# derinworks/penr-oz-neural-network-v3-torch-ddp

Hardware: AMD Instinct MI355X
Metric: tokens/sec (whole node) GPT-2 124M DDP train at 1/2/4/8 MI355X (higher is better)
Workload: dtype bf16; 1 GPU; model=gpt2-124m, global_batch=64, seq_len=1024, micro_batch_per_gpu=64, parallelism=dp1

## Files before the change

### csrc/bindings.cpp

```cpp
#include <torch/extension.h>
#include <hip/hip_runtime.h>
#include <tuple>
#include <vector>

void layernorm_fwd(torch::Tensor x, torch::Tensor w, torch::Tensor b, double eps, torch::Tensor y, torch::Tensor mean,
                   torch::Tensor rstd);
void add_layernorm_fwd(torch::Tensor resid_in, torch::Tensor delta, torch::Tensor resid_out, torch::Tensor w,
                       torch::Tensor b, double eps, torch::Tensor y, torch::Tensor mean, torch::Tensor rstd,
                       c10::optional<torch::Tensor> delta_bias, double dropout_p, int64_t dropout_seed);
void layernorm_bwd(torch::Tensor dy, torch::Tensor x, torch::Tensor mean, torch::Tensor rstd, torch::Tensor w,
                   torch::Tensor dresid, bool accumulate, c10::optional<torch::Tensor> dresid_bf, torch::Tensor dw,
                   torch::Tensor db, c10::optional<torch::Tensor> dbias_prev, double dropout_p, int64_t dropout_seed);
std::vector<torch::Tensor> rmsnorm_fwd(torch::Tensor x, torch::Tensor w, double eps);
std::vector<torch::Tensor> rmsnorm_bwd(torch::Tensor dy, torch::Tensor x, torch::Tensor w, torch::Tensor rstd);
std::vector<torch::Tensor> rms_residual(torch::Tensor x, torch::Tensor a, c10::optional<torch::Tensor> w1,
                                        c10::optional<torch::Tensor> w2, int64_t mode, double eps1, double eps2);
void gelu_fwd(torch::Tensor x, int64_t approx, torch::Tensor y);
void gelu_bwd(torch::Tensor dy, torch::Tensor x, int64_t approx, c10::optional<torch::Tensor> dbias, torch::Tensor out);
void colsum(torch::Tensor x, torch::Tensor out);
torch::Tensor gated_act_fwd(torch::Tensor g, torch::Tensor u, int64_t kind);
torch::Tensor gated_act_packed(torch::Tensor gu, int64_t kind, c10::optional<torch::Tensor> out);
std::vector<torch::Tensor> gated_act_bwd(torch::Tensor dy, torch::Tensor g, torch::Tensor u, int64_t kind);
void gated_act_bwd_packed(torch::Tensor dy, torch::Tensor gu, torch::Tensor dgu, int64_t kind);
void gemma_combine_fwd(int64_t mode, torch::Tensor x, c10::optional<torch::Tensor> a, c10::optional<torch::Tensor> w1,
// ... 88 lines not shown
std::tuple<torch::Tensor, torch::Tensor, torch::Tensor> token_logprobs(torch::Tensor logits, torch::Tensor tokens,
                                                                       int64_t n);
void token_logprobs_step(torch::Tensor logits, torch::Tensor idx, torch::Tensor step, torch::Tensor n_t,
                         torch::Tensor lp_buf, torch::Tensor top_id_buf, torch::Tensor top_lp_buf,
                         torch::Tensor workspace);
void stop_begin(torch::Tensor tail, torch::Tensor n_gen, torch::Tensor done, torch::Tensor finish_at);
void stop_observe(torch::Tensor seqs, torch::Tensor seq_len, torch::Tensor n_seqs, torch::Tensor tail,
                  torch::Tensor n_gen, torch::Tensor done, torch::Tensor finish_at, torch::Tensor tok);
void stop_step(torch::Tensor seqs, torch::Tensor seq_len, torch::Tensor n_seqs, torch::Tensor tail,
               torch::Tensor n_gen, torch::Tensor done, torch::Tensor finish_at, torch::Tensor idx,
               torch::Tensor out_buf, torch::Tensor step);
void logit_bias_apply(torch::Tensor logits, torch::Tensor ids, torch::Tensor bias, torch::Tensor until,
                      torch::Tensor n_entries, c10::optional<torch::Tensor> allow, bool allow_on, torch::Tensor base_t,
                      c10::optional<torch::Tensor> step_t);
std::tuple<int64_t, int64_t, int64_t> logit_bias_plan(int64_t B, int64_t V, bool allow_on);
torch::Tensor update_moments(std::vector<torch::Tensor> ws, std::vector<torch::Tensor> ps);
bool gemm_nt_supported(int64_t M, int64_t N, int64_t K);
void gemm_nt(torch::Tensor a, torch::Tensor b, c10::optional<torch::Tensor> bias, torch::Tensor out,
             c10::optional<torch::Tensor> act, int64_t approx, int64_t group_m, int64_t grid, int64_t ablate);
void wgrad_gemm(torch::Tensor dy, torch::Tensor x, torch::Tensor grad, int64_t tile, int64_t variant, bool accumulate);
void flash_attn_fwd(torch::Tensor qkv, torch::Tensor out, torch::Tensor lse, int64_t H, int64_t Hkv, int64_t D,
                    double scale, double p_drop, int64_t seed);
int64_t flash_fwd_variant(int64_t v);
void flash_bwd_stamps(c10::optional<torch::Tensor> buf);
void flash_attn_bwd(torch::Tensor dout, torch::Tensor qkv, torch::Tensor out, torch::Tensor lse, torch::Tensor dqkv,
                    int64_t H, int64_t Hkv, int64_t D, double scale, double p_drop, int64_t seed,
                    c10::optional<torch::Tensor> dbias);
void flash_attn_gen_fwd(torch::Tensor qkv, torch::Tensor out, torch::Tensor lse, int64_t H, int64_t Hkv, int64_t D,
                        double scale, double p_drop, int64_t seed);
void flash_attn_gen_bwd(torch::Tensor dout, torch::Tensor qkv, torch::Tensor out, torch::Tensor lse,
                        torch::Tensor dqkv, int64_t H, int64_t Hkv, int64_t D, double scale, double p_drop,
                        int64_t seed);
std::vector<int64_t> attn_work_plan(int64_t nblk, int64_t nvh, int64_t slots, int64_t BM, int64_t BN, int64_t T,
                                    int64_t D, double tile_us);

static int64_t cu_masked_stream(int64_t device, std::vector<int64_t> mask) {
  std::vector<uint32_t> m(mask.begin(), mask.end());
  int prev = 0;
  TORCH_CHECK(hipGetDevice(&prev) == hipSuccess, "hipGetDevice failed");
  TORCH_CHECK(hipSetDevice((int)device) == hipSuccess, "hipSetDevice failed");
  hipStream_t st = nullptr;
  const hipError_t e = hipExtStreamCreateWithCUMask(&st, (uint32_t)m.size(), m.data());
  (void)hipSetDevice(prev);
  TORCH_CHECK(e == hipSuccess, "hipExtStreamCreateWithCUMask: ", hipGetErrorString(e));
  return reinterpret_cast<int64_t>(st);
}
// ... 174 lines not shown
        pybind11::arg("nrot") = 0, pybind11::arg("cos") = pybind11::none(), pybind11::arg("sin") = pybind11::none(),
        pybind11::arg("pairs_per_wave") = 0,
        "paired-row int8-weight decode GEMV for 1..4 rows: gated MLP (mode 1) or RoPE QKV (mode 2) epilogue");
  m.def("decode_gemv_q8_limits", &decode_gemv_q8_limits,
        "(rows, K, LN-mode K, paired-row K, K multiple) limits of decode_gemv_q8 / decode_gemv_q8_pair (host only)");
  m.def("decode_gemv_q8_plan", &decode_gemv_q8_plan, pybind11::arg("M"), pybind11::arg("N"), pybind11::arg("K"),
        pybind11::arg("ln") = false, pybind11::arg("rows_per_wave") = 0,
        "decode_gemv_q8's launch plan: (form 0 half-wave / 1 wave-per-row / 2 LN, rows, row pairs per wave, "
        "chunks per lane, grid) (host only)");
  m.def("decode_gemv_q8_pair_plan", &decode_gemv_q8_pair_plan, pybind11::arg("N"), pybind11::arg("K"),
        pybind11::arg("pairs_per_wave") = 0,
        "decode_gemv_q8_pair's launch plan: (pairs per wave, chunks per lane, grid) (host only)");
  m.def("update_moments", &update_moments, "per-epoch weight-update diagnostics: [n, 2] (std(w - prev), std(w))");
  m.def("gemm_nt_supported", &gemm_nt_supported, "shapes the native NT GEMM takes (M % 256, N % 128, K % 32, K >= 160)");
  m.def("gemm_nt", &gemm_nt, pybind11::arg("a"), pybind11::arg("b"), pybind11::arg("bias"), pybind11::arg("out"),
        pybind11::arg("act") = pybind11::none(), pybind11::arg("approx") = 0, pybind11::arg("group_m") = 0,
        pybind11::arg("grid") = 0, pybind11::arg("ablate") = 0,
        "out = a·bᵀ (+ bias) (bf16, both operands reduction-contiguous); with act: act = GELU(out)");
  m.def("wgrad_gemm", &wgrad_gemm, pybind11::arg("dy"), pybind11::arg("x"), pybind11::arg("grad"),
        pybind11::arg("tile") = 256, pybind11::arg("variant") = 8, pybind11::arg("accumulate") = true,
        "grad (+)= dyᵀ·x (fp32 gradient, bf16 operands); accumulate=False overwrites grad");
  m.def("flash_attn_fwd", &flash_attn_fwd);
  m.def("flash_fwd_variant", &flash_fwd_variant, pybind11::arg("variant") = 0,
        "select the forward kernel (1 single-stage, 2 tile-pipelined); returns the previous one");
  m.def("flash_attn_bwd", &flash_attn_bwd, pybind11::arg("dout"), pybind11::arg("qkv"), pybind11::arg("out"),
        pybind11::arg("lse"), pybind11::arg("dqkv"), pybind11::arg("H"), pybind11::arg("Hkv"), pybind11::arg("D"),
        pybind11::arg("scale"), pybind11::arg("p_drop"), pybind11::arg("seed"), pybind11::arg("dbias") = pybind11::none(),
        "causal flash-attention backward (head_dim 64) into dqkv; dbias += column sums of dqkv when given");
  m.def("cu_masked_stream", &cu_masked_stream, "stream restricted to a CU mask (raw hipStream_t)");
  m.def("cu_count", &cu_count, "compute units of a device");
  m.def("flash_bwd_stamps", &flash_bwd_stamps, pybind11::arg("buf") = pybind11::none(),
        "diagnostic: s_memtime phase sums of the dK/dV kernel into an int64 [6] GPU tensor (None: off)");
  m.def("flash_attn_gen_fwd", &flash_attn_gen_fwd, "causal flash attention forward, head_dim 128 / 256");
  m.def("flash_attn_gen_bwd", &flash_attn_gen_bwd, "causal flash attention backward, head_dim 128 / 256");
}
```

### csrc/kernels/flash_attn.hip

```cpp
#include "attn_common.h"
#include <cstdlib>
#include "deferred.h"
#include <type_traits>
#include <torch/extension.h>
#include <ATen/hip/HIPContext.h>

namespace penroz {

constexpr int kD = 64;

template <bool DROPOUT>
__global__ void __launch_bounds__(256, 2) fa_fwd_kernel(const bf16* __restrict__ qkv, bf16* __restrict__ out,
                                                     float* __restrict__ lse, int T, int H, int Hkv, float scale,
                                                     float p_drop, uint64_t seed) {
  constexpr int BM = 128, BN = 64;
  __shared__ __attribute__((aligned(16))) char smem[2][2][BN * 128];
  const int nqb = (T + BM - 1) / BM;
  int qi, bh;
  xcd_head_block(qi, bh);
  const int qb = nqb - 1 - qi;
  const int b = bh / H, h = bh % H, hk = h / (H / Hkv);
  const int lane = threadIdx.x & 63, w = wave_id(), hh = lane >> 5;
  const size_t RS = (size_t)(H + 2 * Hkv) * kD;
  const bf16* qbase = qkv + (size_t)b * T * RS + (size_t)h * kD;
  const bf16* kbase = qkv + (size_t)b * T * RS + (size_t)(H + hk) * kD;
// ... 108 lines not shown
        for (int ss = 0; ss < 2; ++ss) {
          const uint4 pf = acc_frag(s[kh], ss);
#pragma unroll
          for (int dh = 0; dh < 2; ++dh) o[dh] = mfma32(tr_frag(Vt, 32 * kh + 16 * ss, 32 * dh, lane), pf, o[dh]);
        }
    }
    if (j + 1 < ntiles) lstore((j + 1) & 1);
    __syncthreads();
  }
  l = halves_sum(l);
  const float inv = l > 0.f ? 1.f / l : 0.f;
  if (qrow < T) {
    bf16* orow = out + ((size_t)b * T + qrow) * H * kD + (size_t)h * kD;
#pragma unroll
    for (int dh = 0; dh < 2; ++dh)
#pragma unroll
      for (int g = 0; g < 4; ++g)
        store4(orow + 32 * dh + 8 * g + 4 * hh, o[dh][4 * g] * inv, o[dh][4 * g + 1] * inv, o[dh][4 * g + 2] * inv,
               o[dh][4 * g + 3] * inv);
    if (hh == 0) lse[((size_t)b * H + h) * T + qrow] = (m + log2f(l)) * kLn2;
  }
}

template <bool DROPOUT>
__global__ void __launch_bounds__(128, 2) fa_fwd3_kernel(const bf16* __restrict__ qkv, bf16* __restrict__ out,
                                                      float* __restrict__ lse, int T, int H, int Hkv, float scale,
                                                      float p_drop, uint64_t seed) {
  constexpr int BM = 128, BN = 64;
  __shared__ __attribute__((aligned(16))) char smem[2][2][BN * 128];
  const int nqb = (T + BM - 1) / BM;
  int qi, bh;
  xcd_head_block(qi, bh);
  const int qb = nqb - 1 - qi;
  const int b = bh / H, h = bh % H, hk = h / (H / Hkv);
  const int lane = threadIdx.x & 63, w = wave_id(), hh = lane >> 5;
  const size_t RS = (size_t)(H + 2 * Hkv) * kD;
  const bf16* qbase = qkv + (size_t)b * T * RS + (size_t)h * kD;
  const bf16* kbase = qkv + (size_t)b * T * RS + (size_t)(H + hk) * kD;
  const bf16* vbase = qkv + (size_t)b * T * RS + (size_t)(H + Hkv + hk) * kD;
  const int q0 = qb * BM + 64 * w;
  const float c = scale * kLog2e;
  const float inv_keep = DROPOUT ? 1.f / (1.f - p_drop) : 1.f;
  int qrow[2];
  qrow[0] = q0 + (lane & 31);
  qrow[1] = q0 + 32 + (lane & 31);

  uint4 qf[2][4];
#pragma unroll
  for (int a = 0; a < 2; ++a)
#pragma unroll
    for (int s = 0; s < 4; ++s)
      qf[a][s] = qrow[a] < T ? *reinterpret_cast<const uint4*>(qbase + (size_t)qrow[a] * RS + 16 * s + 8 * hh) : zero4();
#pragma unroll
  for (int a = 0; a < 2; ++a)
#pragma unroll
    for (int s = 0; s < 4; ++s) launder(qf[a][s]);

  const unsigned RSB = (unsigned)RS * 2;
  const unsigned k_voff = (unsigned)lane * RSB;
  unsigned v_voff[2];
#pragma unroll
  for (int par = 0; par < 2; ++par) {
    const int row = 8 * par + (lane >> 3);
    const int ch = (lane & 7) ^ ((((row >> 1) & 1) << 2) | ((row >> 2) & 3));
    v_voff[par] = (unsigned)(lane >> 3) * RSB + 16u * ch;
  }
  unsigned vto[2][2];
#pragma unroll
  for (int dh = 0; dh < 2; ++dh)
#pragma unroll
    for (int jj = 0; jj < 2; ++jj) {
      const int col = 32 * dh + 16 * ((lane >> 4) & 1) + 4 * (lane & 3);
      vto[dh][jj] = (unsigned)(tile_off(4 * hh + ((lane & 15) >> 2) + 8 * jj, col >> 3) + ((col & 4) << 1));
    }
  auto vfrag = [&](const char* t, int dh) -> uint4 {
    const s16x4 x = __builtin_amdgcn_ds_read_tr16_b64_v4i16((lds_s16x4*)(t + vto[dh][0]));
    const s16x4 y = __builtin_amdgcn_ds_read_tr16_b64_v4i16((lds_s16x4*)(t + vto[dh][1]));
    const uint2 ux = __builtin_bit_cast(uint2, x), uy = __builtin_bit_cast(uint2, y);
    return uint4{ux.x, ux.y, uy.x, uy.y};
  };
  auto dma = [&](int kt0, int buf) {
    const unsigned dst = __builtin_amdgcn_readfirstlane(lds_addr_of(smem[buf][w]));
    if (kt0 + BN <= T) {
      if (w == 0) {
        const char* sb = reinterpret_cast<const char*>(kbase + (size_t)kt0 * RS);
#pragma unroll
        for (int p = 0; p < 8; ++p) glds16_s(sb + 16 * p, k_voff, dst + p * 1024);
      } else {
#pragma unroll
        for (int p = 0; p < 8; ++p)
          glds16_s(reinterpret_cast<const char*>(vbase + (size_t)(kt0 + 8 * p) * RS), v_voff[p & 1],
                      dst + p * 1024);
      }
    } else if (w == 0) {
      const bf16* g = kbase + (size_t)min(kt0 + lane, T - 1) * RS;
#pragma unroll
      for (int p = 0; p < 8; ++p) glds16(g + 8 * p, dst + p * 1024);
    } else {
      const int prow = lane >> 3, pch = lane & 7;
#pragma unroll
      for (int p = 0; p < 8; ++p) {
        const int row = 8 * p + prow;
        const int ch = pch ^ ((((row >> 1) & 1) << 2) | ((row >> 2) & 3));
        glds16(vbase + (size_t)min(kt0 + row, T - 1) * RS + 8 * ch, dst + p * 1024);
      }
    }
  };

  const int kend = min(T, qb * BM + BM);
  const int ntiles = (kend + BN - 1) / BN;
  const int jlast = min(ntiles - 1, q0 / BN);
  f32x16 o[2][2];
#pragma unroll
  for (int a = 0; a < 2; ++a)
#pragma unroll
    for (int dh = 0; dh < 2; ++dh)
#pragma unroll
      for (int i = 0; i < 16; ++i) o[a][dh][i] = 0.f;
  float m[2] = {-1e30f, -1e30f}, l[2] = {0.f, 0.f};

  auto softmax = [&](auto mask_tag, int a, int kt0, f32x16 (&sa)[2]) {
    constexpr bool MASK = decltype(mask_tag)::value;
    float tmax = -INFINITY;
#pragma unroll
    for (int kh = 0; kh < 2; ++kh)
#pragma unroll
      for (int i = 0; i < 16; ++i) {
// ... 123 lines not shown
  const int row = gid >> 3, part = gid & 7;
  const bool ok = row < B * T * H;
  float s = 0.f;
  if (ok) {
    float a[8], o[8];
    Vec8<bf16>::load(dout + (size_t)row * kD + 8 * part, a);
    Vec8<bf16>::load(out + (size_t)row * kD + 8 * part, o);
#pragma unroll
    for (int k = 0; k < 8; ++k) s += a[k] * o[k];
  }
  s += __shfl_xor(s, 1, 64);
  s += __shfl_xor(s, 2, 64);
  s += __shfl_xor(s, 4, 64);
  if (ok && part == 0) {
    const int h = row % H, t = (row / H) % T, b = row / (H * T);
    delta[((size_t)b * H + h) * T + t] = s;
  }
}

template <int NST>
struct RingWait {
  template <int PER>
  static __device__ __forceinline__ void wait() {
    static_assert(NST >= 3 && NST <= 4 && (PER == 4 || PER == 5), "ring depth / pieces");
    if constexpr (NST == 3) {
      if constexpr (PER == 4) asm volatile("s_waitcnt vmcnt(4)" ::: "memory");
      else asm volatile("s_waitcnt vmcnt(5)" ::: "memory");
    } else {
      if constexpr (PER == 4) asm volatile("s_waitcnt vmcnt(8)" ::: "memory");
      else asm volatile("s_waitcnt vmcnt(10)" ::: "memory");
    }
  }
};

template <typename F, int... S>
__device__ __forceinline__ void ring_unroll(F&& f, int base, std::integer_sequence<int, S...>) {
  (f(base + S, std::integral_constant<int, S>{}), ...);
}
template <typename F, int... S>
__device__ __forceinline__ void ring_tail(F&& f, int base, int total, std::integer_sequence<int, S...>) {
  ((base + S < total ? f(base + S, std::integral_constant<int, S>{}) : void()), ...);
}

__device__ __forceinline__ uint32_t bf16_hilo(float x) {
  const float hi = __bfloat162float(__float2bfloat16(x));
  return pack_bf16x2(hi, x - hi);
}

template <bool DROPOUT, int NST, int GC, bool STAMP = false>
__global__ void __launch_bounds__(256, 2) fa_bwd_dkdv3_kernel(const bf16* __restrict__ qkv,
                                                              const bf16* __restrict__ dout,
                                                              const float* __restrict__ lse,
                                                              const float* __restrict__ delta,
                                                              bf16* __restrict__ dqkv, float* __restrict__ cpart, int T, int H, int Hkv,
                                                              float scale, float p_drop, uint64_t seed,
                                                              unsigned long long* __restrict__ stamps = nullptr,
                                                              int diag = 0) {
  unsigned long long st_acc[5] = {0, 0, 0, 0, 0}, st_n = 0, st_t = 0;
  auto stamp = [&](int seg) {
    if constexpr (STAMP) {
      __builtin_amdgcn_sched_barrier(0);
      const unsigned long long now = __builtin_amdgcn_s_memtime();
      if (seg >= 0) st_acc[seg] += now - st_t;
      st_t = now;
      __builtin_amdgcn_sched_barrier(0);
    }
  };
  constexpr int BK = 128, QS = 64;
  constexpr int TILE = QS * 128;
  constexpr int STAGE = 2 * TILE + 512;
  __shared__ __attribute__((aligned(16))) char smem[NST * STAGE];
  int kb, bh;
  xcd_head_block(kb, bh);
  const int b = bh / Hkv, hk = bh % Hkv;
  const int G = GC ? GC : H / Hkv;
  const int lane = threadIdx.x & 63, w = wave_id(), hh = lane >> 5;
  const size_t RS = (size_t)(H + 2 * Hkv) * kD;
  const size_t ORS = (size_t)H * kD;
  const int kw0 = kb * BK + 32 * w;
  const int key = kw0 + (lane & 31);
  const uint32_t dkey = DROPOUT ? dropout_seedmix(seed) ^ ((uint32_t)(key >> 1) * kDropKeyMul) : 0u;
  const uint32_t dthr = dropout_thr(p_drop);
  const float c = scale * kLog2e;
  const float inv_keep = DROPOUT ? 1.f / (1.f - p_drop) : 1.f;

  const bf16* kbase = qkv + (size_t)b * T * RS + (size_t)(H + hk) * kD;
  const bf16* vbase = qkv + (size_t)b * T * RS + (size_t)(H + Hkv + hk) * kD;
  uint4 kf[4], vf[4];
#pragma unroll
  for (int s = 0; s < 4; ++s) {
    kf[s] = key < T ? *reinterpret_cast<const uint4*>(kbase + (size_t)key * RS + 16 * s + 8 * hh) : zero4();
// ... 17 lines not shown
  unsigned ro[4], to[2][2];
#pragma unroll
  for (int s = 0; s < 4; ++s) ro[s] = (unsigned)tile_off(lane & 31, 2 * s + hh);
#pragma unroll
  for (int dh = 0; dh < 2; ++dh)
#pragma unroll
    for (int j = 0; j < 2; ++j) {
      const int col = 32 * dh + 16 * ((lane >> 4) & 1) + 4 * (lane & 3);
      to[dh][j] = (unsigned)(tile_off(4 * hh + ((lane & 15) >> 2) + 8 * j, col >> 3) + ((col & 4) << 1));
    }
  auto rowf = [&](const char* t, int s) -> uint4 { return *reinterpret_cast<const uint4*>(t + ro[s]); };
  auto trf = [&](const char* t, int dh) -> uint4 {
    const s16x4 x = __builtin_amdgcn_ds_read_tr16_b64_v4i16((lds_s16x4*)(t + to[dh][0]));
    const s16x4 y = __builtin_amdgcn_ds_read_tr16_b64_v4i16((lds_s16x4*)(t + to[dh][1]));
    const uint2 ux = __builtin_bit_cast(uint2, x), uy = __builtin_bit_cast(uint2, y);
    return uint4{ux.x, ux.y, uy.x, uy.y};
  };

  const int s_first = (kb * BK) / QS;
  const int nslices = (T + QS - 1) / QS;
  const int per_head = nslices - s_first;
  const int total = G * per_head;

  const int is_do = w >> 1, half_sel = w & 1;
  const unsigned rsb = (unsigned)(is_do ? ORS : RS) * 2;
  unsigned voff[2];
#pragma unroll
  for (int par = 0; par < 2; ++par) {
    const int row = 8 * par + (lane >> 3);
    const int ch = (lane & 7) ^ ((((row >> 1) & 1) << 2) | ((row >> 2) & 3));
    voff[par] = (unsigned)(lane >> 3) * rsb + 16u * ch;
  }
  auto dma = [&](int it) {
    if (STAMP && diag == 2) return;
    const int itc = (STAMP && diag == 1) ? 0 : min(it, total - 1);
    const int hq = GC == 1 ? hk : hk * G + itc / per_head;
    const int qs0 = (s_first + (GC == 1 ? itc : itc % per_head)) * QS;
    const unsigned st = __builtin_amdgcn_readfirstlane(lds_addr_of(smem + (it % NST) * STAGE));
    const bf16* src = is_do ? dout + (size_t)b * T * ORS + (size_t)hq * kD : qkv + (size_t)b * T * RS + (size_t)hq * kD;
    const size_t rs = is_do ? ORS : RS;
    const unsigned dst = st + is_do * TILE + half_sel * 4096;
    if (qs0 + QS <= T) {
#pragma unroll
      for (int i = 0; i < 4; ++i) {
        const int p = 4 * half_sel + i;
        glds16_s(reinterpret_cast<const char*>(src + (size_t)(qs0 + 8 * p) * rs), voff[p & 1], dst + i * 1024);
      }
    } else {
#pragma unroll
      for (int i = 0; i < 4; ++i) {
        const int p = 4 * half_sel + i;
        const int row = 8 * p + (lane >> 3);
        const int ch = (lane & 7) ^ ((((row >> 1) & 1) << 2) | ((row >> 2) & 3));
        glds16(src + (size_t)min(qs0 + row, T - 1) * rs + 8 * ch, dst + i * 1024);
      }
    }
    if (w < 2) {
      const float* sp = (w == 0 ? lse : delta) + ((size_t)b * H + hq) * T + min(qs0 + lane, T - 1);
      glds4(sp, st + 2 * TILE + 256 * w);
    }
  };
  auto wait_next = [&]() {
    if (w < 2)
      RingWait<NST>::template wait<5>();
    else
      RingWait<NST>::template wait<4>();
  };
  if (total > 0) {
#pragma unroll
    for (int i = 0; i < NST - 1; ++i) dma(i);
    wait_next();
  }
  __syncthreads();
  auto iter = [&](int it, auto stage_tag) {
    constexpr int ST = decltype(stage_tag)::value;
    stamp(-1);
    dma(it + NST - 1);
    stamp(0);
    const char* stg = smem + ST * STAGE;
    const float* lse_s = reinterpret_cast<const float*>(stg + 2 * TILE);
    const float* del_s = lse_s + QS;
    const int hq = GC == 1 ? hk : hk * G + it / per_head;
    const int qs0 = (s_first + (GC == 1 ? it : it % per_head)) * QS;
    bool act[2];
    f32x16 sp[2], dp[2];
#pragma unroll
    for (int half = 0; half < 2; ++half) {
      const int qh0 = qs0 + 32 * half;
      act[half] = qh0 + 31 >= kw0 && kw0 < T && qh0 < T;
// ... 80 lines not shown
            dk[dh] = mfma32(HOIST ? tqq[ss][dh] : trf(Qt + 16 * ss * 128, dh), sf, dk[dh]);
          }
        }
      }
    }
    stamp(2);
    wait_next();
    stamp(3);
    __syncthreads();
    stamp(4);
    if constexpr (STAMP) ++st_n;
  };
  int it = 0;
  for (; it + NST <= total; it += NST) ring_unroll(iter, it, std::make_integer_sequence<int, NST>{});
  ring_tail(iter, it, total, std::make_integer_sequence<int, NST - 1>{});
  asm volatile("s_waitcnt vmcnt(0)" ::: "memory");
  if constexpr (STAMP) {
    if (lane == 0) {
#pragma unroll
      for (int i = 0; i < 5; ++i) atomicAdd(stamps + i, st_acc[i]);
      atomicAdd(stamps + 5, st_n);
    }
  }
  if (cpart != nullptr) {
    float* prow = cpart + (((size_t)b * gridDim.x + kb) * 4 + w) * RS;
    colsum32_wave(dk, scale, key < T, prow + (size_t)(H + hk) * kD);
    colsum32_wave(dv, 1.f, key < T, prow + (size_t)(H + Hkv + hk) * kD);
  }
  if (key < T) {
    bf16* dkrow = dqkv + ((size_t)b * T + key) * RS + (size_t)(H + hk) * kD;
    bf16* dvrow = dqkv + ((size_t)b * T + key) * RS + (size_t)(H + Hkv + hk) * kD;
#pragma unroll
    for (int dh = 0; dh < 2; ++dh)
#pragma unroll
      for (int g = 0; g < 4; ++g) {
        const int d = 32 * dh + 8 * g + 4 * hh;
        store4(dkrow + d, dk[dh][4 * g] * scale, dk[dh][4 * g + 1] * scale, dk[dh][4 * g + 2] * scale,
               dk[dh][4 * g + 3] * scale);
        store4(dvrow + d, dv[dh][4 * g], dv[dh][4 * g + 1], dv[dh][4 * g + 2], dv[dh][4 * g + 3]);
      }
  }
}

template <bool DROPOUT, int NST>
__global__ void __launch_bounds__(256, 2) fa_bwd_dq4_kernel(const bf16* __restrict__ qkv, const bf16* __restrict__ dout,
                                                        const float* __restrict__ lse,
                                                        float* __restrict__ delta, bf16* __restrict__ dqkv, float* __restrict__ cpart,
                                                        int T, int H, int Hkv, float scale, float p_drop,
                                                        uint64_t seed, const bf16* __restrict__ out) {
  constexpr int BM = 128, BN = 64;
  __shared__ __attribute__((aligned(16))) char smem[NST][2][BN * 128];
  const int nqb = (T + BM - 1) / BM;
  int qi, bh;
  xcd_head_block(qi, bh);
  const int qb = nqb - 1 - qi;
  const int b = bh / H, h = bh % H, hk = h / (H / Hkv);
  const int lane = threadIdx.x & 63, w = wave_id(), hh = lane >> 5;
  const size_t RS = (size_t)(H + 2 * Hkv) * kD;
  const size_t ORS = (size_t)H * kD;
  const bf16* kbase = qkv + (size_t)b * T * RS + (size_t)(H + hk) * kD;
  const bf16* vbase = qkv + (size_t)b * T * RS + (size_t)(H + Hkv + hk) * kD;
  const int q0 = qb * BM + 32 * w;
  const int qrow = q0 + (lane & 31);
  const uint32_t drow = DROPOUT ? dropout_seedmix(seed) ^ ((uint32_t)((b * H + h) * T + qrow) * kDropRowMul) : 0u;
  const uint32_t dthr = dropout_thr(p_drop);
  const float c = scale * kLog2e;
  const float inv_keep = DROPOUT ? 1.f / (1.f - p_drop) : 1.f;

  uint4 qf[4], dof[4];
  const bool qok = qrow < T;
#pragma unroll
  for (int s = 0; s < 4; ++s) {
    qf[s] = qok ? *reinterpret_cast<const uint4*>(qkv + (size_t)b * T * RS + (size_t)h * kD + (size_t)qrow * RS + 16 * s +
// ... 20 lines not shown
                 __uint_as_float(ow[k] & 0xffff0000u) * __uint_as_float(dw[k] & 0xffff0000u);
      }
    }
    sum += __shfl_xor(sum, 32, 64);
    dl = sum;
    if (qok && hh == 0) delta[rr] = sum;
  } else {
    dl = qok ? delta[rr] : 0.f;
  }
#pragma unroll
  for (int s = 0; s < 4; ++s) {
    qf[s] = scale_bf16x8(qf[s], c);
    launder(qf[s]);
    launder(dof[s]);
  }
  asm volatile("" : "+v"(l2), "+v"(dl));
  f32x16 s_init, dp_init;
#pragma unroll
  for (int i = 0; i < 16; ++i) {
    s_init[i] = -l2;
    dp_init[i] = DROPOUT ? 0.f : -dl;
  }

  const int is_v = w >> 1, half_sel = w & 1;
  const unsigned RSB = (unsigned)RS * 2;
  unsigned voff[2];
#pragma unroll
  for (int par = 0; par < 2; ++par) {
    const int row = 8 * par + (lane >> 3);
    const int ch = (lane & 7) ^ ((((row >> 1) & 1) << 2) | ((row >> 2) & 3));
    voff[par] = (unsigned)(lane >> 3) * RSB + 16u * ch;
  }
  const bf16* dsrc = is_v ? vbase : kbase;
  const int kend = min(T, qb * BM + BM);
  const int ntiles = (kend + BN - 1) / BN;
  f32x16 dq[2];
#pragma unroll
  for (int dh = 0; dh < 2; ++dh)
#pragma unroll
    for (int i = 0; i < 16; ++i) dq[dh][i] = 0.f;

  unsigned ro[4], to[2][2];
#pragma unroll
  for (int s = 0; s < 4; ++s) ro[s] = (unsigned)tile_off(lane & 31, 2 * s + hh);
#pragma unroll
  for (int dh = 0; dh < 2; ++dh)
#pragma unroll
    for (int j = 0; j < 2; ++j) {
      const int col = 32 * dh + 16 * ((lane >> 4) & 1) + 4 * (lane & 3);
      to[dh][j] = (unsigned)(tile_off(4 * hh + ((lane & 15) >> 2) + 8 * j, col >> 3) + ((col & 4) << 1));
    }
  auto rowf = [&](const char* t, int s) -> uint4 { return *reinterpret_cast<const uint4*>(t + ro[s]); };
  auto trf = [&](const char* t, int dh) -> uint4 {
    const s16x4 x = __builtin_amdgcn_ds_read_tr16_b64_v4i16((lds_s16x4*)(t + to[dh][0]));
    const s16x4 y = __builtin_amdgcn_ds_read_tr16_b64_v4i16((lds_s16x4*)(t + to[dh][1]));
    const uint2 ux = __builtin_bit_cast(uint2, x), uy = __builtin_bit_cast(uint2, y);
    return uint4{ux.x, ux.y, uy.x, uy.y};
  };
  auto dma = [&](int jt) {
    const int kt0 = min(jt, ntiles - 1) * BN;
    const unsigned dst = __builtin_amdgcn_readfirstlane(lds_addr_of(smem[jt % NST][is_v])) + half_sel * 4096;
    if (kt0 + BN <= T) {
#pragma unroll
      for (int i = 0; i < 4; ++i) {
        const int p = 4 * half_sel + i;
        glds16_s(reinterpret_cast<const char*>(dsrc + (size_t)(kt0 + 8 * p) * RS), voff[p & 1], dst + i * 1024);
      }
    } else {
#pragma unroll
      for (int i = 0; i < 4; ++i) {
        const int p = 4 * half_sel + i;
        const int row = 8 * p + (lane >> 3);
        const int ch = (lane & 7) ^ ((((row >> 1) & 1) << 2) | ((row >> 2) & 3));
        glds16(dsrc + (size_t)min(kt0 + row, T - 1) * RS + 8 * ch, dst + i * 1024);
      }
    }
  };
#pragma unroll
  for (int i = 0; i < NST - 1; ++i) dma(i);
  RingWait<NST>::template wait<4>();
  __syncthreads();
  auto iter = [&](int j, auto stage_tag) {
    constexpr int ST = decltype(stage_tag)::value;
    const int kt0 = j * BN;
    dma(j + NST - 1);
    const char* Kt = smem[ST][0];
    const char* Vt = smem[ST][1];
    if (kt0 <= q0 + 31) {
      f32x16 s[2], dp[2];
#pragma unroll
      for (int kh = 0; kh < 2; ++kh) {
        uint4 ka[4], va[4];
#pragma unroll
        for (int st = 0; st < 4; ++st) {
          ka[st] = rowf(Kt + 32 * kh * 128, st);
          va[st] = rowf(Vt + 32 * kh * 128, st);
        }
        s[kh] = mfma32(ka[0], qf[0], s_init);
        dp[kh] = mfma32(va[0], dof[0], dp_init);
#pragma unroll
        for (int st = 1; st < 4; ++st) {
          s[kh] = mfma32(ka[st], qf[st], s[kh]);
          dp[kh] = mfma32(va[st], dof[st], dp[kh]);
// ... 16 lines not shown
            float p = fexp2(s[kh][i]);
            if constexpr (MASK) p = (k > qrow || k >= T || !qok) ? 0.f : p;
            if constexpr (DROPOUT) {
              const uint32_t km = kpair0 + (uint32_t)(16 * kh + 4 * (i >> 2) + ((i & 3) >> 1)) * kDropKeyMul;
              const bool keep = dropout_keep_mixed(drow, km, (i & 1) != 0, dthr);
              s[kh][i] = p * ((keep ? dp[kh][i] * inv_keep : 0.f) - dl);
            } else {
              s[kh][i] = p * dp[kh][i];
            }
          }
        };
        if (need_mask)
          grads(std::true_type{});
        else
          grads(std::false_type{});
#pragma unroll
        for (int ss = 0; ss < 2; ++ss) {
          const uint4 sf = acc_frag(s[kh], ss);
#pragma unroll
          for (int dh = 0; dh < 2; ++dh) dq[dh] = mfma32(tk[ss][dh], sf, dq[dh]);
        }
      }
    }
    RingWait<NST>::template wait<4>();
    __syncthreads();
  };
  int j = 0;
  for (; j + NST <= ntiles; j += NST) ring_unroll(iter, j, std::make_integer_sequence<int, NST>{});
  ring_tail(iter, j, ntiles, std::make_integer_sequence<int, NST - 1>{});
  asm volatile("s_waitcnt vmcnt(0)" ::: "memory");
  if (cpart != nullptr)
    colsum32_wave(dq, scale, qok, cpart + (((size_t)b * nqb + qb) * 4 + w) * RS + (size_t)h * kD);
  if (qok) {
    bf16* dqrow = dqkv + ((size_t)b * T + qrow) * RS + (size_t)h * kD;
#pragma unroll
    for (int dh = 0; dh < 2; ++dh)
#pragma unroll
      for (int g = 0; g < 4; ++g)
        store4(dqrow + 32 * dh + 8 * g + 4 * hh, dq[dh][4 * g] * scale, dq[dh][4 * g + 1] * scale,
               dq[dh][4 * g + 2] * scale, dq[dh][4 * g + 3] * scale);
  }
}

}

using namespace penroz;

static void check_qkv(const torch::Tensor& qkv, int64_t H, int64_t Hkv, int64_t D) {
  TORCH_CHECK(qkv.is_cuda() && qkv.is_contiguous() && qkv.dim() == 3, "qkv must be a contiguous [B, T, W] GPU tensor");
  TORCH_CHECK(qkv.scalar_type() == torch::kBFloat16, "flash attention expects bf16");
  TORCH_CHECK(D == kD, "flash attention kernel is built for head_dim 64");
  TORCH_CHECK(H % Hkv == 0 && qkv.size(2) == (H + 2 * Hkv) * D, "qkv width must be (H + 2*Hkv)*D");
}

static int g_fa_fwd_variant = 3;

void flash_attn_fwd(torch::Tensor qkv, torch::Tensor out, torch::Tensor lse, int64_t H, int64_t Hkv, int64_t D,
                    double scale, double p_drop, int64_t seed) {
  check_qkv(qkv, H, Hkv, D);
  const int B = qkv.size(0), T = qkv.size(1);
  TORCH_CHECK(out.is_contiguous() && out.scalar_type() == torch::kBFloat16 && out.numel() == (int64_t)B * T * H * D);
  TORCH_CHECK(lse.is_contiguous() && lse.scalar_type() == torch::kFloat32 && lse.numel() == (int64_t)B * H * T);
  if (B == 0 || T == 0) return;
  dim3 grid((T + 127) / 128, B * H);
  auto stream = at::hip::getCurrentHIPStream();
  const bf16* q = reinterpret_cast<const bf16*>(qkv.data_ptr());
  bf16* o = reinterpret_cast<bf16*>(out.data_ptr());
  if (p_drop > 0.0)
    hipLaunchKernelGGL(fa_fwd_kernel<true>, grid, dim3(256), 0, stream, q, o, lse.data_ptr<float>(), T, (int)H,
                       (int)Hkv, (float)scale, (float)p_drop, (uint64_t)seed);
  else if (g_fa_fwd_variant == 1)
    hipLaunchKernelGGL(fa_fwd_kernel<false>, grid, dim3(256), 0, stream, q, o, lse.data_ptr<float>(), T, (int)H,
                       (int)Hkv, (float)scale, 0.f, (uint64_t)seed);
  else
    hipLaunchKernelGGL(fa_fwd3_kernel<false>, grid, dim3(128), 0, stream, q, o, lse.data_ptr<float>(), T, (int)H,
                       (int)Hkv, (float)scale, 0.f, (uint64_t)seed);
}

int64_t flash_fwd_variant(int64_t v) {
  const int64_t prev = g_fa_fwd_variant;
  if (v > 0) g_fa_fwd_variant = (int)v;
  return prev;
}

static unsigned long long* g_fa_stamps = nullptr;
void flash_bwd_stamps(c10::optional<torch::Tensor> buf) {
  if (buf.has_value() && buf->defined()) {
    TORCH_CHECK(buf->is_cuda() && buf->scalar_type() == torch::kInt64 && buf->numel() >= 6 && buf->is_contiguous());
    g_fa_stamps = reinterpret_cast<unsigned long long*>(buf->data_ptr());
  } else {
    g_fa_stamps = nullptr;
  }
}

void flash_attn_bwd(torch::Tensor dout, torch::Tensor qkv, torch::Tensor out, torch::Tensor lse, torch::Tensor dqkv,
                    int64_t H, int64_t Hkv, int64_t D, double scale, double p_drop, int64_t seed,
                    c10::optional<torch::Tensor> dbias) {
  check_qkv(qkv, H, Hkv, D);
  const int B = qkv.size(0), T = qkv.size(1);
  TORCH_CHECK(dout.is_contiguous() && dout.scalar_type() == torch::kBFloat16 && dout.numel() == (int64_t)B * T * H * D);
  TORCH_CHECK(out.is_contiguous() && out.numel() == dout.numel());
  TORCH_CHECK(dqkv.is_contiguous() && dqkv.scalar_type() == torch::kBFloat16 && dqkv.numel() == qkv.numel());
  if (B == 0 || T == 0) return;
  auto delta = torch::empty({B, H, T}, qkv.options().dtype(torch::kFloat32));
// ... 6 lines not shown
    const int rows = B * T * H;
    hipLaunchKernelGGL(fa_bwd_pre_kernel, dim3((rows * 8 + 255) / 256), dim3(256), 0, stream,
                       reinterpret_cast<const bf16*>(dout.data_ptr()), reinterpret_cast<const bf16*>(out.data_ptr()),
                       delta.data_ptr<float>(), B, T, (int)H);
  }
  const bf16* q = reinterpret_cast<const bf16*>(qkv.data_ptr());
  const bf16* d = reinterpret_cast<const bf16*>(dout.data_ptr());
  bf16* g = reinterpret_cast<bf16*>(dqkv.data_ptr());
  dim3 gkv((T + 127) / 128, B * Hkv), gq((T + 127) / 128, B * H);
  using BwdKernel = void (*)(const bf16*, const bf16*, const float*, const float*, bf16*, float*, int, int, int, float, float,
                            uint64_t, unsigned long long*, int);
  using DqKernel = void (*)(const bf16*, const bf16*, const float*, float*, bf16*, float*, int, int, int, float, float,
                            uint64_t, const bf16*);
  const bool drop = p_drop > 0.0;
  BwdKernel kv;
  DqKernel dq;
  if (H == Hkv && !drop && g_fa_stamps)
    kv = fa_bwd_dkdv3_kernel<false, 3, 1, true>;
  else if (H == Hkv)
    kv = drop ? fa_bwd_dkdv3_kernel<true, 3, 1> : fa_bwd_dkdv3_kernel<false, 3, 1>;
  else
    kv = drop ? fa_bwd_dkdv3_kernel<true, 3, 0> : fa_bwd_dkdv3_kernel<false, 3, 0>;
  dq = drop ? fa_bwd_dq4_kernel<true, 3> : fa_bwd_dq4_kernel<false, 3>;
  const float pd = drop ? (float)p_drop : 0.f;
  static const int kv_diag = [] {
    const char* e = std::getenv("PENROZ_FA_STAMP_DIAG");
    return e ? std::atoi(e) : 0;
  }();
  const bool want_bias = dbias.has_value() && dbias->defined();
  const int W = (int)((H + 2 * Hkv) * D), nblk = (T + 127) / 128;
  if (want_bias)
    TORCH_CHECK(dbias->is_cuda() && dbias->scalar_type() == torch::kFloat32 && dbias->is_contiguous() &&
                    dbias->numel() == W, "dbias must be a contiguous fp32 [(H + 2*Hkv)*D] GPU tensor");
  torch::Tensor part;
  if (want_bias) part = torch::empty({(int64_t)B * nblk * 4, W}, qkv.options().dtype(torch::kFloat32));
  float* pp = want_bias ? part.data_ptr<float>() : nullptr;
  hipLaunchKernelGGL(dq, gq, dim3(256), 0, stream, q, d, lse.data_ptr<float>(), delta.data_ptr<float>(), g, pp, T,
                     (int)H, (int)Hkv, (float)scale, pd, (uint64_t)seed,
                     prepass ? nullptr : reinterpret_cast<const bf16*>(out.data_ptr()));
  hipLaunchKernelGGL(kv, gkv, dim3(256), 0, stream, q, d, lse.data_ptr<float>(), delta.data_ptr<float>(), g, pp, T,
                     (int)H, (int)Hkv, (float)scale, pd, (uint64_t)seed, g_fa_stamps, kv_diag);
  if (want_bias) {
    float* outs[1] = {dbias->data_ptr<float>()};
    reduce_partials_auto(part, 1, B * nblk * 4, W, outs, stream);
  }
}
```

Measured before the change: 1.057 million tokens/s.

## Widen flash-attention workgroups so more waves share each K/V staging ring

Templates the forward and backward flash-attention kernels on waves per workgroup, so 4-wave forward and 8-wave backward workgroups cover larger query/key blocks while splitting the LDS DMA pieces across more waves. The forward default switches to the 4-wave variant. The backward 8-wave variants are opt-in through an environment variable or binding and default to 4 waves. The aim is more reuse of each staged K/V (or Q/dO) tile per workgroup and less global-to-LDS traffic per query row. The cost is fewer workgroups in the grid and heavier per-workgroup synchronisation, and the colsum partial indexing is reworked to match.

Result: no change. 1.065 million tokens/s (median of 6 runs) (+0.8%).

```diff
diff --git a/csrc/bindings.cpp b/csrc/bindings.cpp
--- a/csrc/bindings.cpp
+++ b/csrc/bindings.cpp
@@ -134,6 +134,7 @@
 void flash_attn_fwd(torch::Tensor qkv, torch::Tensor out, torch::Tensor lse, int64_t H, int64_t Hkv, int64_t D,
                     double scale, double p_drop, int64_t seed);
 int64_t flash_fwd_variant(int64_t v);
+std::tuple<int64_t, int64_t> flash_bwd_variant(int64_t dq, int64_t dkdv);
 void flash_bwd_stamps(c10::optional<torch::Tensor> buf);
 void flash_attn_bwd(torch::Tensor dout, torch::Tensor qkv, torch::Tensor out, torch::Tensor lse, torch::Tensor dqkv,
                     int64_t H, int64_t Hkv, int64_t D, double scale, double p_drop, int64_t seed,
@@ -354,7 +355,11 @@
         "grad (+)= dyᵀ·x (fp32 gradient, bf16 operands); accumulate=False overwrites grad");
   m.def("flash_attn_fwd", &flash_attn_fwd);
   m.def("flash_fwd_variant", &flash_fwd_variant, pybind11::arg("variant") = 0,
-        "select the forward kernel (1 single-stage, 2 tile-pipelined); returns the previous one");
+        "select the D=64 forward kernel (1 single-stage, 3 two query blocks per wave, 4 the same with 4 waves per "
+        "workgroup); 0 only queries; returns the previous one");
+  m.def("flash_bwd_variant", &flash_bwd_variant, pybind11::arg("dq") = 0, pybind11::arg("dkdv") = 0,
+        "select the D=64 backward kernels' workgroup width, per kernel (1: 4 waves, 2: 8 waves sharing each ring, "
+        "0 keeps); returns the previous (dq, dkdv)");
   m.def("flash_attn_bwd", &flash_attn_bwd, pybind11::arg("dout"), pybind11::arg("qkv"), pybind11::arg("out"),
         pybind11::arg("lse"), pybind11::arg("dqkv"), pybind11::arg("H"), pybind11::arg("Hkv"), pybind11::arg("D"),
         pybind11::arg("scale"), pybind11::arg("p_drop"), pybind11::arg("seed"), pybind11::arg("dbias") = pybind11::none(),
diff --git a/csrc/kernels/flash_attn.hip b/csrc/kernels/flash_attn.hip
--- a/csrc/kernels/flash_attn.hip
+++ b/csrc/kernels/flash_attn.hip
@@ -1,6 +1,8 @@
 #include "attn_common.h"
 #include <cstdlib>
 #include "deferred.h"
+#include <initializer_list>
+#include <tuple>
 #include <type_traits>
 #include <torch/extension.h>
 #include <ATen/hip/HIPContext.h>
@@ -155,11 +157,13 @@
   }
 }
 
-template <bool DROPOUT>
-__global__ void __launch_bounds__(128, 2) fa_fwd3_kernel(const bf16* __restrict__ qkv, bf16* __restrict__ out,
+template <bool DROPOUT, int NW = 2>
+__global__ void __launch_bounds__(64 * NW, 2) fa_fwd3_kernel(const bf16* __restrict__ qkv, bf16* __restrict__ out,
                                                       float* __restrict__ lse, int T, int H, int Hkv, float scale,
                                                       float p_drop, uint64_t seed) {
-  constexpr int BM = 128, BN = 64;
+  static_assert(NW == 2 || NW == 4, "waves per workgroup");
+  constexpr int BM = 64 * NW, BN = 64;
+  constexpr int PP = 16 / NW;
   __shared__ __attribute__((aligned(16))) char smem[2][2][BN * 128];
   const int nqb = (T + BM - 1) / BM;
   int qi, bh;
@@ -167,6 +171,7 @@
   const int qb = nqb - 1 - qi;
   const int b = bh / H, h = bh % H, hk = h / (H / Hkv);
   const int lane = threadIdx.x & 63, w = wave_id(), hh = lane >> 5;
+  const int is_v = w / (NW / 2), p0 = PP * (w % (NW / 2));
   const size_t RS = (size_t)(H + 2 * Hkv) * kD;
   const bf16* qbase = qkv + (size_t)b * T * RS + (size_t)h * kD;
   const bf16* kbase = qkv + (size_t)b * T * RS + (size_t)(H + hk) * kD;
@@ -213,29 +218,30 @@
     return uint4{ux.x, ux.y, uy.x, uy.y};
   };
   auto dma = [&](int kt0, int buf) {
-    const unsigned dst = __builtin_amdgcn_readfirstlane(lds_addr_of(smem[buf][w]));
+    const unsigned dst = __builtin_amdgcn_readfirstlane(lds_addr_of(smem[buf][is_v])) + p0 * 1024;
     if (kt0 + BN <= T) {
-      if (w == 0) {
-        const char* sb = reinterpret_cast<const char*>(kbase + (size_t)kt0 * RS);
-#pragma unroll
-        for (int p = 0; p < 8; ++p) glds16_s(sb + 16 * p, k_voff, dst + p * 1024);
+      if (is_v == 0) {
+        const char* sb = reinterpret_cast<const char*>(kbase + (size_t)kt0 * RS) + 16 * p0;
+#pragma unroll
+        for (int i = 0; i < PP; ++i) glds16_s(sb + 16 * i, k_voff, dst + i * 1024);
       } else {
 #pragma unroll
-        for (int p = 0; p < 8; ++p)
-          glds16_s(reinterpret_cast<const char*>(vbase + (size_t)(kt0 + 8 * p) * RS), v_voff[p & 1],
-                      dst + p * 1024);
-      }
-    } else if (w == 0) {
-      const bf16* g = kbase + (size_t)min(kt0 + lane, T - 1) * RS;
-#pragma unroll
-      for (int p = 0; p < 8; ++p) glds16(g + 8 * p, dst + p * 1024);
+        for (int i = 0; i < PP; ++i)
+          glds16_s(reinterpret_cast<const char*>(vbase + (size_t)(kt0 + 8 * (p0 + i)) * RS), v_voff[i & 1],
+                      dst + i * 1024);
+      }
+    } else if (is_v == 0) {
+      const bf16* g = kbase + (size_t)min(kt0 + lane, T - 1) * RS + 8 * p0;
+#pragma unroll
+      for (int i = 0; i < PP; ++i) glds16(g + 8 * i, dst + i * 1024);
     } else {
       const int prow = lane >> 3, pch = lane & 7;
 #pragma unroll
-      for (int p = 0; p < 8; ++p) {
+      for (int i = 0; i < PP; ++i) {
+        const int p = p0 + i;
         const int row = 8 * p + prow;
         const int ch = pch ^ ((((row >> 1) & 1) << 2) | ((row >> 2) & 3));
-        glds16(vbase + (size_t)min(kt0 + row, T - 1) * RS + 8 * ch, dst + p * 1024);
+        glds16(vbase + (size_t)min(kt0 + row, T - 1) * RS + 8 * ch, dst + i * 1024);
       }
     }
   };
@@ -405,14 +411,8 @@
 struct RingWait {
   template <int PER>
   static __device__ __forceinline__ void wait() {
-    static_assert(NST >= 3 && NST <= 4 && (PER == 4 || PER == 5), "ring depth / pieces");
-    if constexpr (NST == 3) {
-      if constexpr (PER == 4) asm volatile("s_waitcnt vmcnt(4)" ::: "memory");
-      else asm volatile("s_waitcnt vmcnt(5)" ::: "memory");
-    } else {
-      if constexpr (PER == 4) asm volatile("s_waitcnt vmcnt(8)" ::: "memory");
-      else asm volatile("s_waitcnt vmcnt(10)" ::: "memory");
-    }
+    static_assert(NST >= 3 && NST <= 4 && PER >= 2 && PER <= 5, "ring depth / pieces");
+    asm volatile("s_waitcnt vmcnt(%0)" ::"n"((NST - 2) * PER) : "memory");
   }
 };
 
@@ -430,8 +430,8 @@
   return pack_bf16x2(hi, x - hi);
 }
 
-template <bool DROPOUT, int NST, int GC, bool STAMP = false>
-__global__ void __launch_bounds__(256, 2) fa_bwd_dkdv3_kernel(const bf16* __restrict__ qkv,
+template <bool DROPOUT, int NST, int GC, bool STAMP = false, int NW = 4>
+__global__ void __launch_bounds__(64 * NW, 2) fa_bwd_dkdv3_kernel(const bf16* __restrict__ qkv,
                                                               const bf16* __restrict__ dout,
                                                               const float* __restrict__ lse,
                                                               const float* __restrict__ delta,
@@ -449,7 +449,9 @@
       __builtin_amdgcn_sched_barrier(0);
     }
   };
-  constexpr int BK = 128, QS = 64;
+  static_assert(NW == 4 || (NW == 8 && !DROPOUT && !STAMP), "waves per workgroup");
+  constexpr int BK = 32 * NW, QS = 64;
+  constexpr int PP = 16 / NW;
   constexpr int TILE = QS * 128;
   constexpr int STAGE = 2 * TILE + 512;
   __shared__ __attribute__((aligned(16))) char smem[NST * STAGE];
@@ -513,7 +515,7 @@
   const int per_head = nslices - s_first;
   const int total = G * per_head;
 
-  const int is_do = w >> 1, half_sel = w & 1;
+  const int is_do = w >> (NW == 4 ? 1 : 2), p0 = PP * (w & (NW / 2 - 1));
   const unsigned rsb = (unsigned)(is_do ? ORS : RS) * 2;
   unsigned voff[2];
 #pragma unroll
@@ -530,17 +532,17 @@
     const unsigned st = __builtin_amdgcn_readfirstlane(lds_addr_of(smem + (it % NST) * STAGE));
     const bf16* src = is_do ? dout + (size_t)b * T * ORS + (size_t)hq * kD : qkv + (size_t)b * T * RS + (size_t)hq * kD;
     const size_t rs = is_do ? ORS : RS;
-    const unsigned dst = st + is_do * TILE + half_sel * 4096;
+    const unsigned dst = st + is_do * TILE + p0 * 1024;
     if (qs0 + QS <= T) {
 #pragma unroll
-      for (int i = 0; i < 4; ++i) {
-        const int p = 4 * half_sel + i;
+      for (int i = 0; i < PP; ++i) {
+        const int p = p0 + i;
         glds16_s(reinterpret_cast<const char*>(src + (size_t)(qs0 + 8 * p) * rs), voff[p & 1], dst + i * 1024);
       }
     } else {
 #pragma unroll
-      for (int i = 0; i < 4; ++i) {
-        const int p = 4 * half_sel + i;
+      for (int i = 0; i < PP; ++i) {
+        const int p = p0 + i;
         const int row = 8 * p + (lane >> 3);
         const int ch = (lane & 7) ^ ((((row >> 1) & 1) << 2) | ((row >> 2) & 3));
         glds16(src + (size_t)min(qs0 + row, T - 1) * rs + 8 * ch, dst + i * 1024);
@@ -553,9 +555,9 @@
   };
   auto wait_next = [&]() {
     if (w < 2)
-      RingWait<NST>::template wait<5>();
+      RingWait<NST>::template wait<PP + 1>();
     else
-      RingWait<NST>::template wait<4>();
+      RingWait<NST>::template wait<PP>();
   };
   if (total > 0) {
 #pragma unroll
@@ -682,8 +684,9 @@
       atomicAdd(stamps + 5, st_n);
     }
   }
-  if (cpart != nullptr) {
-    float* prow = cpart + (((size_t)b * gridDim.x + kb) * 4 + w) * RS;
+  const int nsl = (T + 127) / 128 * 4, sl = kb * NW + w;
+  if (cpart != nullptr && sl < nsl) {
+    float* prow = cpart + ((size_t)b * nsl + sl) * RS;
     colsum32_wave(dk, scale, key < T, prow + (size_t)(H + hk) * kD);
     colsum32_wave(dv, 1.f, key < T, prow + (size_t)(H + Hkv + hk) * kD);
   }
@@ -702,13 +705,15 @@
   }
 }
 
-template <bool DROPOUT, int NST>
-__global__ void __launch_bounds__(256, 2) fa_bwd_dq4_kernel(const bf16* __restrict__ qkv, const bf16* __restrict__ dout,
+template <bool DROPOUT, int NST, int NW = 4>
+__global__ void __launch_bounds__(64 * NW, 2) fa_bwd_dq4_kernel(const bf16* __restrict__ qkv, const bf16* __restrict__ dout,
                                                         const float* __restrict__ lse,
                                                         float* __restrict__ delta, bf16* __restrict__ dqkv, float* __restrict__ cpart,
                                                         int T, int H, int Hkv, float scale, float p_drop,
                                                         uint64_t seed, const bf16* __restrict__ out) {
-  constexpr int BM = 128, BN = 64;
+  static_assert(NW == 4 || (NW == 8 && !DROPOUT), "waves per workgroup");
+  constexpr int BM = 32 * NW, BN = 64;
+  constexpr int PP = 16 / NW;
   __shared__ __attribute__((aligned(16))) char smem[NST][2][BN * 128];
   const int nqb = (T + BM - 1) / BM;
   int qi, bh;
@@ -775,7 +780,7 @@
     dp_init[i] = DROPOUT ? 0.f : -dl;
   }
 
-  const int is_v = w >> 1, half_sel = w & 1;
+  const int is_v = w >> (NW == 4 ? 1 : 2), p0 = PP * (w & (NW / 2 - 1));
   const unsigned RSB = (unsigned)RS * 2;
   unsigned voff[2];
 #pragma unroll
@@ -812,17 +817,17 @@
   };
   auto dma = [&](int jt) {
     const int kt0 = min(jt, ntiles - 1) * BN;
-    const unsigned dst = __builtin_amdgcn_readfirstlane(lds_addr_of(smem[jt % NST][is_v])) + half_sel * 4096;
+    const unsigned dst = __builtin_amdgcn_readfirstlane(lds_addr_of(smem[jt % NST][is_v])) + p0 * 1024;
     if (kt0 + BN <= T) {
 #pragma unroll
-      for (int i = 0; i < 4; ++i) {
-        const int p = 4 * half_sel + i;
+      for (int i = 0; i < PP; ++i) {
+        const int p = p0 + i;
         glds16_s(reinterpret_cast<const char*>(dsrc + (size_t)(kt0 + 8 * p) * RS), voff[p & 1], dst + i * 1024);
       }
     } else {
 #pragma unroll
-      for (int i = 0; i < 4; ++i) {
-        const int p = 4 * half_sel + i;
+      for (int i = 0; i < PP; ++i) {
+        const int p = p0 + i;
         const int row = 8 * p + (lane >> 3);
         const int ch = (lane & 7) ^ ((((row >> 1) & 1) << 2) | ((row >> 2) & 3));
         glds16(dsrc + (size_t)min(kt0 + row, T - 1) * RS + 8 * ch, dst + i * 1024);
@@ -831,7 +836,7 @@
   };
 #pragma unroll
   for (int i = 0; i < NST - 1; ++i) dma(i);
-  RingWait<NST>::template wait<4>();
+  RingWait<NST>::template wait<PP>();
   __syncthreads();
   auto iter = [&](int j, auto stage_tag) {
     constexpr int ST = decltype(stage_tag)::value;
@@ -894,15 +899,16 @@
         }
       }
     }
-    RingWait<NST>::template wait<4>();
+    RingWait<NST>::template wait<PP>();
     __syncthreads();
   };
   int j = 0;
   for (; j + NST <= ntiles; j += NST) ring_unroll(iter, j, std::make_integer_sequence<int, NST>{});
   ring_tail(iter, j, ntiles, std::make_integer_sequence<int, NST - 1>{});
   asm volatile("s_waitcnt vmcnt(0)" ::: "memory");
-  if (cpart != nullptr)
-    colsum32_wave(dq, scale, qok, cpart + (((size_t)b * nqb + qb) * 4 + w) * RS + (size_t)h * kD);
+  const int nsl = (T + 127) / 128 * 4, sl = qb * NW + w;
+  if (cpart != nullptr && sl < nsl)
+    colsum32_wave(dq, scale, qok, cpart + ((size_t)b * nsl + sl) * RS + (size_t)h * kD);
   if (qok) {
     bf16* dqrow = dqkv + ((size_t)b * T + qrow) * RS + (size_t)h * kD;
 #pragma unroll
@@ -925,7 +931,20 @@
   TORCH_CHECK(H % Hkv == 0 && qkv.size(2) == (H + 2 * Hkv) * D, "qkv width must be (H + 2*Hkv)*D");
 }
 
-static int g_fa_fwd_variant = 3;
+static int fa_env_choice(const char* name, int dflt, std::initializer_list<int> allowed) {
+  const char* e = std::getenv(name);
+  if (!e || !*e) return dflt;
+  const int v = std::atoi(e);
+  for (int a : allowed)
+    if (a == v) return v;
+  TORCH_CHECK(false, name, "=", e, " is not one of the supported values");
+  return dflt;
+}
+
+static int& fa_fwd_variant_ref() {
+  static int v = fa_env_choice("PENROZ_FA_FWD_VARIANT", 4, {1, 3, 4});
+  return v;
+}
 
 void flash_attn_fwd(torch::Tensor qkv, torch::Tensor out, torch::Tensor lse, int64_t H, int64_t Hkv, int64_t D,
                     double scale, double p_drop, int64_t seed) {
@@ -941,17 +960,36 @@
   if (p_drop > 0.0)
     hipLaunchKernelGGL(fa_fwd_kernel<true>, grid, dim3(256), 0, stream, q, o, lse.data_ptr<float>(), T, (int)H,
                        (int)Hkv, (float)scale, (float)p_drop, (uint64_t)seed);
-  else if (g_fa_fwd_variant == 1)
+  else if (fa_fwd_variant_ref() == 1)
     hipLaunchKernelGGL(fa_fwd_kernel<false>, grid, dim3(256), 0, stream, q, o, lse.data_ptr<float>(), T, (int)H,
                        (int)Hkv, (float)scale, 0.f, (uint64_t)seed);
+  else if (fa_fwd_variant_ref() == 4)
+    hipLaunchKernelGGL((fa_fwd3_kernel<false, 4>), dim3((T + 255) / 256, B * H), dim3(256), 0, stream, q, o,
+                       lse.data_ptr<float>(), T, (int)H, (int)Hkv, (float)scale, 0.f, (uint64_t)seed);
   else
     hipLaunchKernelGGL(fa_fwd3_kernel<false>, grid, dim3(128), 0, stream, q, o, lse.data_ptr<float>(), T, (int)H,
                        (int)Hkv, (float)scale, 0.f, (uint64_t)seed);
 }
 
 int64_t flash_fwd_variant(int64_t v) {
-  const int64_t prev = g_fa_fwd_variant;
-  if (v > 0) g_fa_fwd_variant = (int)v;
+  const int64_t prev = fa_fwd_variant_ref();
+  if (v > 0) fa_fwd_variant_ref() = (int)v;
+  return prev;
+}
+
+static int& fa_dq_variant_ref() {
+  static int v = fa_env_choice("PENROZ_FA_DQ_WAVES", 4, {4, 8}) / 4;
+  return v;
+}
+static int& fa_dkdv_variant_ref() {
+  static int v = fa_env_choice("PENROZ_FA_DKDV_WAVES", 4, {4, 8}) / 4;
+  return v;
+}
+std::tuple<int64_t, int64_t> flash_bwd_variant(int64_t dq, int64_t dkdv) {
+  TORCH_CHECK(dq >= 0 && dq <= 2 && dkdv >= 0 && dkdv <= 2, "flash_bwd_variant: 0 (keep), 1 (4 waves) or 2 (8 waves)");
+  const std::tuple<int64_t, int64_t> prev{fa_dq_variant_ref(), fa_dkdv_variant_ref()};
+  if (dq > 0) fa_dq_variant_ref() = (int)dq;
+  if (dkdv > 0) fa_dkdv_variant_ref() = (int)dkdv;
   return prev;
 }
 
@@ -1004,6 +1042,16 @@
   else
     kv = drop ? fa_bwd_dkdv3_kernel<true, 3, 0> : fa_bwd_dkdv3_kernel<false, 3, 0>;
   dq = drop ? fa_bwd_dq4_kernel<true, 3> : fa_bwd_dq4_kernel<false, 3>;
+  const bool wide_dq = fa_dq_variant_ref() == 2 && !drop;
+  const bool wide_kv = fa_dkdv_variant_ref() == 2 && !drop && !g_fa_stamps;
+  if (wide_dq) {
+    dq = fa_bwd_dq4_kernel<false, 3, 8>;
+    gq.x = (T + 255) / 256;
+  }
+  if (wide_kv) {
+    kv = H == Hkv ? fa_bwd_dkdv3_kernel<false, 3, 1, false, 8> : fa_bwd_dkdv3_kernel<false, 3, 0, false, 8>;
+    gkv.x = (T + 255) / 256;
+  }
   const float pd = drop ? (float)p_drop : 0.f;
   static const int kv_diag = [] {
     const char* e = std::getenv("PENROZ_FA_STAMP_DIAG");
@@ -1017,11 +1065,12 @@
   torch::Tensor part;
   if (want_bias) part = torch::empty({(int64_t)B * nblk * 4, W}, qkv.options().dtype(torch::kFloat32));
   float* pp = want_bias ? part.data_ptr<float>() : nullptr;
-  hipLaunchKernelGGL(dq, gq, dim3(256), 0, stream, q, d, lse.data_ptr<float>(), delta.data_ptr<float>(), g, pp, T,
-                     (int)H, (int)Hkv, (float)scale, pd, (uint64_t)seed,
+  hipLaunchKernelGGL(dq, gq, dim3(wide_dq ? 512 : 256), 0, stream, q, d, lse.data_ptr<float>(),
+                     delta.data_ptr<float>(), g, pp, T, (int)H, (int)Hkv, (float)scale, pd, (uint64_t)seed,
                      prepass ? nullptr : reinterpret_cast<const bf16*>(out.data_ptr()));
-  hipLaunchKernelGGL(kv, gkv, dim3(256), 0, stream, q, d, lse.data_ptr<float>(), delta.data_ptr<float>(), g, pp, T,
-                     (int)H, (int)Hkv, (float)scale, pd, (uint64_t)seed, g_fa_stamps, kv_diag);
+  hipLaunchKernelGGL(kv, gkv, dim3(wide_kv ? 512 : 256), 0, stream, q, d, lse.data_ptr<float>(),
+                     delta.data_ptr<float>(), g, pp, T, (int)H, (int)Hkv, (float)scale, pd, (uint64_t)seed, g_fa_stamps,
+                     kv_diag);
   if (want_bias) {
     float* outs[1] = {dbias->data_ptr<float>()};
     reduce_partials_auto(part, 1, B * nblk * 4, W, outs, stream);
```
